# zerchen/AlignSDF

Hardware: AMD Instinct MI355X
Metric: meshes_per_sec_hand_plus_obj_N256 (higher is better)
Workload: dtype f32-class: 2 x f16 planes per operand (22 bit), 3 f16 MFMAs per product sum, f32 accumulate, every voxel <= 1e-5

## Files before the change

### alignsdf_amd/csrc/sdf_mlp_f16w_kernel.h

```cpp
#pragma once
#include "sdf_mlp_f16_kernel.h"

namespace asdf {

static_assert(ASDF16_STAGE_KB == 16 && ASDF16_MIX_SPLIT && ASDF16_EPI_STEPS && ASDF16_DMA_PER_KB && ASDF16_PRELOAD && ASDF16_LOADS_FIRST &&
                  ASDF16_PIN_ACC,
              "the W form is written for the shipped schedule of the split-half kernel");

#define ASDF_MFMA16W(a, b, c) __builtin_amdgcn_mfma_f32_16x16x32_f16((a), (b), (c), 0, 0, 0)
#define ASDF_MFMA4W(a, b, c) __builtin_amdgcn_mfma_f32_16x16x4f32((a), (b), (c), 0, 0, 0)

__device__ __forceinline__ f32x4 acc_get4(const f32x16& a, int o) {
  f32x4 v;
  v[0] = a[o]; v[1] = a[o + 1]; v[2] = a[o + 2]; v[3] = a[o + 3];
  return v;
}
__device__ __forceinline__ void acc_set4(f32x16& a, int o, const f32x4& v) { a[o] = v[0]; a[o + 1] = v[1]; a[o + 2] = v[2]; a[o + 3] = v[3]; }

__device__ __forceinline__ f32x16 load_bias16w(const float* tile_words, int lane) {
  const int q = lane >> 4;
  const float* w0 = tile_words + (q & 1) * 16 + 4 * (q >> 1);
  int dup = 0;
  asm volatile("" : "+v"(dup));
  const float* w1 = w0 + dup;
  f32x16 r;
  acc_set4(r, 0, *reinterpret_cast<const f32x4*>(w0)); acc_set4(r, 4, *reinterpret_cast<const f32x4*>(w0 + 8));
  acc_set4(r, 8, *reinterpret_cast<const f32x4*>(w1)); acc_set4(r, 12, *reinterpret_cast<const f32x4*>(w1 + 8));
  return r;
}

__device__ __forceinline__ void pin_acc_w(f32x16& acc) {
#pragma unroll
  for (int o = 0; o < 16; o += 4) {
    f32x4 q;
    q[0] = acc[o]; q[1] = acc[o + 1]; q[2] = acc[o + 2]; q[3] = acc[o + 3];
    asm volatile("" : "+a"(q));
    acc[o] = q[0]; acc[o + 1] = q[1]; acc[o + 2] = q[2]; acc[o + 3] = q[3];
  }
}

#ifndef ASDF16_W_M0_CLOBBER
#define ASDF16_W_M0_CLOBBER 1
#endif
template <int P>
__device__ __forceinline__ void dma_piece_w(const float* src, unsigned dst) {
#if ASDF16_W_M0_CLOBBER
  asm volatile(
      "s_mov_b32 m0, %1\n\t"
      "s_nop 0\n\t"
      "global_load_lds_dwordx4 %0, off offset:%c2"
      :
      : "v"(src + (P >> 2) * 1024), "s"(dst + (P >> 2) * 4096), "i"((P & 3) * 1024)
      : "memory", "m0");
#else
  dma_piece<P>(src, dst);
#endif
}

template <int KB, int Q, int SLOT, int ABL, class Pre, class Epi>
__device__ __forceinline__ void stage16w(f32x16& acc, const h8 (&xh)[KB], const h8 (&xl)[KB], const float* ring, const float* next_src,
                                         unsigned lds_ring_base, int lane, int wave, h8 (&ah)[S16<2>::kPrefetch], h8 (&al)[S16<2>::kPrefetch],
                                         Pre&& pre, Epi&& epi) {
  using SG = S16<2>;
  constexpr int PF = SG::kPrefetch;
  constexpr int BKB = ASDF16_BARRIER_KB;
  constexpr int nslot = (SLOT + kRing - 1) % kRing;
  static_assert(KB == 32 || KB == 16, "records per tile");
  static_assert(kS16Kb - BKB >= SG::kPieces, "one LDS-DMA piece per record behind the barrier");
  const float* src = next_src + wave * SG::kWaveFloats + lane * 4;
  const unsigned dst = lds_ring_base + (nslot * SG::kFloats + wave * SG::kWaveFloats) * 4;
  const h8* cur = reinterpret_cast<const h8*>(ring + SLOT * SG::kFloats) + lane;
  const h8* nxt = reinterpret_cast<const h8*>(ring + ((SLOT + 1) % kRing) * SG::kFloats) + lane;
  h8 bufh[kS16Kb + PF], bufl[kS16Kb + PF];
#pragma unroll
  for (int i = 0; i < PF; ++i) { bufh[i] = ah[i]; bufl[i] = al[i]; }
#pragma unroll
  for (int kb = 0; kb < kS16Kb; ++kb) {
    if (kb == BKB && !(ABL & 1)) {
      asm volatile("s_waitcnt vmcnt(8)" ::: "memory");
      if (!(ABL & 16)) __builtin_amdgcn_s_barrier();
    }
    bufh[kb + PF] = kb + PF < kS16Kb ? cur[((kb + PF) * 2 + 0) * 64] : nxt[((kb + PF - kS16Kb) * 2 + 0) * 64];
    bufl[kb + PF] = kb + PF < kS16Kb ? cur[((kb + PF) * 2 + 1) * 64] : nxt[((kb + PF - kS16Kb) * 2 + 1) * 64];
    pre(kb);
    __builtin_amdgcn_sched_barrier(0);
    const int ri = Q * kS16Kb + kb;
    const int xb = KB == 32 ? 2 * (ri % 16) : (ri & ~1), o = (KB == 32 ? ri / 16 : (ri & 1)) * 4;
    const bool snake = ri & 1;
    const int xa = xb + (snake ? 1 : 0), xc = xb + (snake ? 0 : 1);
#pragma unroll
    for (int j = 0; j < 3; ++j) {
      f32x4 s0 = acc_get4(acc, o), s1 = acc_get4(acc, 8 + o);
      f32x4& sa = snake ? s1 : s0;
      f32x4& sb = snake ? s0 : s1;
      if (j == 0) { sa = ASDF_MFMA16W(bufh[kb], xl[xa], sa); sa = ASDF_MFMA16W(bufl[kb], xh[xa], sa); }
      if (j == 1) { sa = ASDF_MFMA16W(bufh[kb], xh[xa], sa); sb = ASDF_MFMA16W(bufh[kb], xl[xc], sb); }
      if (j == 2) { sb = ASDF_MFMA16W(bufl[kb], xh[xc], sb); sb = ASDF_MFMA16W(bufh[kb], xh[xc], sb); }
      acc_set4(acc, o, s0); acc_set4(acc, 8 + o, s1);
      const int m = j == 2 ? kb - BKB : -1;
      if (!(ABL & 1) && !(ABL & 32) && m >= 0 && m < SG::kPieces) {
        if (m == 0) dma_piece_w<0>(src, dst);
        else if (m == 1) dma_piece_w<1>(src, dst);
        else if (m == 2) dma_piece_w<2>(src, dst);
        else if (m == 3) dma_piece_w<3>(src, dst);
        else if (m == 4) dma_piece_w<4>(src, dst);
        else if (m == 5) dma_piece_w<5>(src, dst);
        else if (m == 6) dma_piece_w<6>(src, dst);
        else dma_piece_w<7>(src, dst);
        __builtin_amdgcn_sched_barrier(0);
      }
      epi(kb, j);
      __builtin_amdgcn_sched_barrier(0);
    }
    __builtin_amdgcn_sched_barrier(0);
  }
#pragma unroll
  for (int i = 0; i < PF; ++i) { ah[i] = bufh[kS16Kb + i]; al[i] = bufl[kS16Kb + i]; }
}

template <int ABL = 0, bool SUB = false>
__device__ __forceinline__ void sdf_mlp_f16w_body(const DecodeParams& p) {
  using CL = CstLayout<2>;
  using SG = S16<2>;
  static_assert(lds_bytes_f16(2, 2) <= 160 * 1024, "LDS budget");
  extern __shared__ __attribute__((aligned(16))) float smem[];
  float* ring = smem;
  float* cst = smem + SG::kRingFloats;

  const int tid = threadIdx.x;
  const int lane = tid & 63;
  const int wave = __builtin_amdgcn_readfirstlane(tid >> 6);
  const int half = lane >> 5;

  float lat_vs = p.vs, lat_o0 = p.o0, lat_o1 = p.o1, lat_o2 = p.o2;
  if (p.lattice) { lat_o0 = p.lattice[0]; lat_o1 = p.lattice[1]; lat_o2 = p.lattice[2]; lat_vs = p.lattice[3]; }
  long long npts = p.P;
  if (SUB) { const long long c = *p.count_dev; npts = c < npts ? c : npts; }
  const long long ntiles = (npts + kWgPts - 1) / kWgPts;
  if ((long long)blockIdx.x >= ntiles) return;

  const unsigned lds_ring_base = (unsigned)(size_t)(__attribute__((address_space(3))) float*)ring;
  if (!SUB && p.status && p.mode != kPointList && blockIdx.x == 0 && tid == 0) reinterpret_cast<long long*>(p.status + ASDF_STATUS_CLOCK)[0] = clock64();

#pragma unroll 1
  for (int slot = 0; slot < p.num_mlps; ++slot) {
    const int head = p.first_mlp + slot;
    const float* hc = cst;
    int* wrec = reinterpret_cast<int*>(cst + CL::kFloats) + wave * kWrecInts;
    if (lane < kWrecInts) wrec[lane] = lane >= 16 ? 0 : ((lane & 7) < 3 ? 0x7fffffff : ((lane & 7) < 6 ? -1 : 0));
    asm volatile("s_waitcnt vmcnt(0)" ::: "memory");
    __syncthreads();
    {
      const f32x4* src4 = reinterpret_cast<const f32x4*>(p.cst + (size_t)head * CL::kFloats);
      for (int i = tid; i < CL::kFloats / 4; i += 256) reinterpret_cast<f32x4*>(cst)[i] = src4[i];
    }
    const float* sbase0 = p.stream + (size_t)kStagesAll * kStageFloats + (size_t)head * kS16Head * SG::kFloats;
#pragma unroll
    for (int s = 0; s < ((ABL & 33) ? kRing : kRing - 1); ++s) {
      const float* src = sbase0 + (size_t)s * SG::kFloats + wave * SG::kWaveFloats + lane * 4;
      const unsigned dst = lds_ring_base + (s * SG::kFloats + wave * SG::kWaveFloats) * 4;
#pragma unroll
      for (int c = 0; c < SG::kPieces; ++c) lds_dma16(src + c * 256, dst + c * 1024);
    }
    if (ABL & 33) asm volatile("s_waitcnt vmcnt(0)" ::: "memory");
    asm volatile("s_waitcnt vmcnt(16)" ::: "memory");
    __syncthreads();
    h8 ah[SG::kPrefetch], al[SG::kPrefetch];
#pragma unroll
    for (int i = 0; i < SG::kPrefetch; ++i) {
      ah[i] = (reinterpret_cast<const h8*>(ring) + lane)[(i * 2 + 0) * 64];
      al[i] = (reinterpret_cast<const h8*>(ring) + lane)[(i * 2 + 1) * 64];
    }
    const float mul1 = hc[CL::kB4 + 2], mul2 = hc[CL::kB4 + 3], mul0 = hc[CL::kB4 + 4];
    int audit_from = 0x7fffffff;
    if (SUB && p.audit) audit_from = p.audit_from ? *p.audit_from : 0;
    auto bias_at = [&](int off, int t) -> f32x16 { return load_bias16w(hc + off + t * 32, lane); };
    auto pt_word = [&](int off, int t, int fh) -> float {
      return hc[off + (t * 2 + (lane >> 5)) * 64 + ((lane >> 4) & 1) * 32 + 16 * fh + (lane & 15)];
    };

#pragma unroll 1
    for (long long tile = blockIdx.x; tile < ntiles; tile += gridDim.x) {
      const long long pi = tile * kWgPts + wave * kWavePts + (lane & 31);
      const bool valid = pi < npts;
      const long long po = SUB ? (valid ? (long long)p.idx[pi] : 0) : pi;
      float x0 = 0.f, x1 = 0.f, x2 = 0.f;
      if (SUB) {
        grid_point(po, p.N, p.grid_mode, lat_vs, lat_o0, lat_o1, lat_o2, x0, x1, x2);
      } else if (p.mode == kPointList) {
        if (valid) { x0 = p.xyz[pi * 3 + 0]; x1 = p.xyz[pi * 3 + 1]; x2 = p.xyz[pi * 3 + 2]; }
      } else {
        grid_point(valid ? pi : 0, p.N, p.mode, lat_vs, lat_o0, lat_o1, lat_o2, x0, x1, x2);
      }
      float amax = 0.0f, amax1 = 0.0f, amax2 = 0.0f;
      float bq[2];
      {
        const int q = lane >> 4;
#pragma unroll
        for (int g = 0; g < 2; ++g) {
          const int src = (lane & 15) + 16 * g;
          const float c0 = __shfl(x0, src), c1 = __shfl(x1, src), c2 = __shfl(x2, src);
          bq[g] = q == 0 ? c0 : q == 1 ? c1 : q == 2 ? c2 : 0.0f;
        }
      }
      auto pt_mfma = [&](f32x16& a, const float* af) {
#pragma unroll
        for (int fh = 0; fh < 2; ++fh)
#pragma unroll
          for (int g = 0; g < 2; ++g) acc_set4(a, 8 * g + 4 * fh, ASDF_MFMA4W(af[fh], bq[g], acc_get4(a, 8 * g + 4 * fh)));
      };
      const float* sbase = sbase0;
      asm volatile("" : "+s"(sbase));
      auto src_of = [&](int s) -> const float* {
        return sbase + (size_t)(s < kS16Head ? s : s - kS16Head) * SG::kFloats;
      };

      f32x16 acc1[2], acc2[2], acc3[2];
      float pf2[2];
      float w4c[2], w4n[2];
      constexpr int kPreKb = ASDF16_PRE_KB;
      static_assert(kPreKb >= kEpiShift + kEpiChunks, "preload K-block inside the epilogue slots");
      auto load_pf2 = [&](int t) { pf2[0] = pt_word(CL::kA2, t, 0); pf2[1] = pt_word(CL::kA2, t, 1); };
      auto load_w4 = [&](int t, int c) {
        const int wq = lane >> 4;
        const float* w4 = hc + CL::kW4 + (t * 2 + (wq & 1)) * 16 + 4 * (2 * ((c >> 1) & 1) + (wq >> 1)) + 2 * (c & 1);
        w4n[0] = w4[0]; w4n[1] = w4[1];
      };
      auto next_w4 = [&]() { w4c[0] = w4n[0]; w4c[1] = w4n[1]; };

      h8 h0h[2 * kTilesHidden], h0l[2 * kTilesHidden];
      f32x16 acc0[2];
      float pf0[2][2];
      auto l0_load = [&](int t) {
        acc0[t & 1] = bias_at(CL::kC0, t);
        pf0[t & 1][0] = pt_word(CL::kA0, t, 0); pf0[t & 1][1] = pt_word(CL::kA0, t, 1);
      };
      constexpr int kL0Front = kS16Kb / 2;
      l0_load(0);
      acc1[0] = bias_at(CL::kB1, 0);
#pragma unroll
      for (int t = 0; t < kL0Front; ++t) {
        l0_load(t + 1);
        __builtin_amdgcn_sched_barrier(0);
        f32x16 acc = acc0[t & 1];
        pt_mfma(acc, pf0[t & 1]);
        split_tile<2, 1, true>(acc, acc, mul0, h0h[2 * t], h0l[2 * t], h0h[2 * t + 1], h0l[2 * t + 1], amax);
        __builtin_amdgcn_sched_barrier(0);
      }

#define ASDF_STAGE16W(KB, Q, SLOT, ACC, XH, XL, SIDX, PRE, EPI) \
  stage16w<KB, Q, SLOT, ABL>(ACC, XH, XL, ring, src_of((SIDX) + 3), lds_ring_base, lane, wave, ah, al, PRE, EPI)

      float er[2] = {0.0f, 0.0f};
      h8 h1h[2 * kTilesL1], h1l[2 * kTilesL1];
      if (ABL & 4) for (int t = 0; t < 2 * kTilesL1; ++t) { h1h[t] = h0h[t]; h1l[t] = h0l[t]; }
#pragma unroll
      for (int t = 0; t < kTilesL1; ++t) {
        f32x16& acc = acc1[t & 1];
        auto pre = [&](int kb) {
          const int c = kb - kEpiShift;
          if (t == 0 && c >= 0 && c + 1 < kEpiChunks) l0_load(kL0Front + c + 1);
        };
        auto epi = [&](int kb, int g) {
          const int c = kb - kEpiShift;
          if (c < 0 || c >= kEpiChunks) return;
          if (t == 0) {
            const int T = kL0Front + c;
            if (g == 0) pt_mfma(acc0[T & 1], pf0[T & 1]);
#pragma unroll
            for (int e = 0; e < 8; ++e)
              if (e / 3 == g) split_part<2, 1, true>(acc0[T & 1], acc0[T & 1], mul0, h0h[2 * T], h0l[2 * T], h0h[2 * T + 1], h0l[2 * T + 1], amax, e);
            return;
          }
          if (ABL & 4) { asm volatile("" :: "v"(acc1[(t - 1) & 1])); return; }
          if (g == 0) pin_acc_w(acc1[(t - 1) & 1]);
          split_part<2, 1, true>(acc1[(t - 1) & 1], acc1[(t - 1) & 1], mul1, h1h[2 * (t - 1)], h1l[2 * (t - 1)], h1h[2 * (t - 1) + 1],
                                 h1l[2 * (t - 1) + 1], amax1, c, -1, g, er);
        };
        auto pre_last = [&](int c) {
          if (c != kPreKb) return;
          if (t + 1 < kTilesL1) acc1[(t + 1) & 1] = bias_at(CL::kB1, t + 1);
          else { acc2[0] = bias_at(CL::kC2, 0); load_pf2(0); }
        };
        if (t & 1) {
          ASDF_STAGE16W(32, 0, 2, acc, h0h, h0l, t * 2 + 0, pre, epi);
          ASDF_STAGE16W(32, 1, 3, acc, h0h, h0l, t * 2 + 1, pre_last, NoOp16());
        } else {
          ASDF_STAGE16W(32, 0, 0, acc, h0h, h0l, t * 2 + 0, pre, epi);
          ASDF_STAGE16W(32, 1, 1, acc, h0h, h0l, t * 2 + 1, pre_last, NoOp16());
        }
      }

      h8 h2h[2 * kTilesHidden], h2l[2 * kTilesHidden];
      if (ABL & 4) for (int t = 0; t < 2 * kTilesHidden; ++t) { h2h[t] = h0h[t]; h2l[t] = h0l[t]; }
      auto l2_tile = [&](int t, auto slot_tag) {
        constexpr int SLOT = decltype(slot_tag)::value;
        f32x16& acc = acc2[t & 1];
        pt_mfma(acc, pf2);
        auto epi = [&](int kb, int g) {
          const int c = kb - kEpiShift;
          if (c < 0 || c >= kEpiChunks) return;
          if (ABL & 4) { asm volatile("" :: "v"(acc2[(t + 1) & 1]), "v"(acc1[1])); return; }
          if (t > 0) {
            if (g == 0) pin_acc_w(acc2[(t - 1) & 1]);
            split_part<2, 1, true>(acc2[(t - 1) & 1], acc2[(t - 1) & 1], mul2, h2h[2 * (t - 1)], h2l[2 * (t - 1)], h2h[2 * (t - 1) + 1],
                                   h2l[2 * (t - 1) + 1], amax2, c, -1, g, er);
          } else {
            if (g == 0) pin_acc_w(acc1[(kTilesL1 - 1) & 1]);
            split_part<2, 1, true>(acc1[(kTilesL1 - 1) & 1], acc1[(kTilesL1 - 1) & 1], mul1, h1h[2 * kTilesL1 - 2], h1l[2 * kTilesL1 - 2],
                                   h1h[2 * kTilesL1 - 1], h1l[2 * kTilesL1 - 1], amax1, c, -1, g, er);
          }
        };
        auto pre_last = [&](int c) {
          if (c != kPreKb) return;
          if (t + 1 < kTilesHidden) { acc2[(t + 1) & 1] = bias_at(CL::kC2, t + 1); load_pf2(t + 1); }
          else acc3[0] = bias_at(CL::kB3, 0);
        };
        constexpr int S0 = 256 / kS16Kb;
        ASDF_STAGE16W(16, 0, SLOT, acc, h1h, h1l, S0 + t, pre_last, epi);
      };
#pragma unroll
      for (int tt = 0; tt < kTilesHidden / 4; ++tt) {
        l2_tile(4 * tt + 0, std::integral_constant<int, 0>());
        l2_tile(4 * tt + 1, std::integral_constant<int, 1>());
        l2_tile(4 * tt + 2, std::integral_constant<int, 2>());
        l2_tile(4 * tt + 3, std::integral_constant<int, 3>());
      }

      float part = 0.0f, partg = 0.0f;
      auto dot_w4_part = [&](const f32x16& a, int c, int only = -1) {
#pragma unroll
        for (int r = 0; r < 2; ++r) {
          if (only >= 0 && only != r) continue;
          const float v = __int_as_float(max(__float_as_int(a[2 * c + r]), 0));
          if (c < 4) part = fmaf(v, w4c[r], part);
          else partg = fmaf(v, w4c[r], partg);
        }
      };
#pragma unroll
      for (int t = 0; t < kTilesHidden; ++t) {
        f32x16& acc = acc3[t & 1];
        auto pre = [&](int kb) {
          const int c = kb - kEpiShift;
          if (t > 0 && c >= 0 && c + 1 < kEpiChunks) load_w4(t - 1, c + 1);
        };
        auto epi = [&](int kb, int g) {
          const int c = kb - kEpiShift;
          if (c < 0 || c >= kEpiChunks) return;
          if (ABL & 4) { asm volatile("" :: "v"(acc3[(t + 1) & 1]), "v"(acc2[1])); return; }
          if (t > 0) {
            if (g == 0) pin_acc_w(acc3[(t - 1) & 1]);
            if (g < 2) dot_w4_part(acc3[(t - 1) & 1], c, g);
            else next_w4();
          } else {
            if (g == 0) pin_acc_w(acc2[(kTilesHidden - 1) & 1]);
            split_part<2, 1, true>(acc2[(kTilesHidden - 1) & 1], acc2[(kTilesHidden - 1) & 1], mul2, h2h[2 * kTilesHidden - 2],
                                   h2l[2 * kTilesHidden - 2], h2h[2 * kTilesHidden - 1], h2l[2 * kTilesHidden - 1], amax2, c, -1, g, er);
          }
        };
        auto pre_last = [&](int c) {
          if (c != kPreKb) return;
          if (t + 1 < kTilesHidden) acc3[(t + 1) & 1] = bias_at(CL::kB3, t + 1);
          load_w4(t, 0);
          next_w4();
        };
        constexpr int S0 = 512 / kS16Kb;
        if (t & 1) {
          ASDF_STAGE16W(32, 0, 2, acc, h2h, h2l, S0 + t * 2 + 0, pre, epi);
          ASDF_STAGE16W(32, 1, 3, acc, h2h, h2l, S0 + t * 2 + 1, pre_last, NoOp16());
        } else {
          ASDF_STAGE16W(32, 0, 0, acc, h2h, h2l, S0 + t * 2 + 0, pre, epi);
          ASDF_STAGE16W(32, 1, 1, acc, h2h, h2l, S0 + t * 2 + 1, pre_last, NoOp16());
        }
      }
#pragma unroll
      for (int c = 0; c < kEpiChunks; ++c) {
        if (c + 1 < kEpiChunks) load_w4(kTilesHidden - 1, c + 1);
        dot_w4_part(acc3[(kTilesHidden - 1) & 1], c);
        next_w4();
      }
#undef ASDF_STAGE16W
      part += __shfl_xor(part, 16); partg += __shfl_xor(partg, 16);
      part += __shfl_xor(part, 32); partg += __shfl_xor(partg, 32);
      part = (lane & 16) ? partg : part;
      const float pre = part + hc[CL::kB4];
      const float sdf = tanhf(pre);
      const bool is_hand = head == 0;
      if (SUB) {
        int dm = 0, da = 0, flips = 0, na = 0;
        float sq = 0.0f;
        if (valid && half == 0) {
          const bool aud = p.audit && pi >= (long long)audit_from;
          float* out = is_hand ? p.sdf0 : p.sdf1;
          if (out) {
            const float before = out[po];
            const int d = __float_as_int(fabsf(sdf - before));
            if (aud) { da = max(da, d); flips += ((before < 0.0f) != (sdf < 0.0f)) ? 1 : 0; ++na; sq += (sdf - before) * (sdf - before); }
            else dm = max(dm, d);
            if (!aud || p.audit_from) out[po] = sdf;
          }
        }
#pragma unroll
        for (int m = 32; m >= 1; m >>= 1) {
          dm = max(dm, __shfl_xor(dm, m)); da = max(da, __shfl_xor(da, m));
          flips += __shfl_xor(flips, m); na += __shfl_xor(na, m);
          if (p.audit) sq += __shfl_xor(sq, m);
        }
        if (lane == 0) {
          if (p.status && dm) atomicMax(p.status + ASDF_STATUS_MAX_ERR, dm);
          if (p.audit && na) {
            atomicMax(p.audit + kAuditMaxErr, da); if (flips) atomicAdd(p.audit + kAuditFlips, flips); atomicAdd(p.audit + kAuditEvals, na);
            atomicAdd(reinterpret_cast<float*>(p.audit + kAuditSumSq), sq);
          }
        }
      } else if (valid && half == 0) {
        float* out = is_hand ? p.sdf0 : p.sdf1;
        if (out) out[po] = sdf;
      }
      amax *= mul0; amax1 *= mul1; amax2 *= mul2;
      const bool act_over = !(fmaxf(amax, fmaxf(amax1, amax2)) < 65504.0f);
      const int bad = (valid && (act_over || !(fabsf(sdf) <= 1.0f))) ? 1 : 0;
      if (p.status) {
        const int m0 = wave_max_i32(valid ? __float_as_int(amax) : 0), m1 = wave_max_i32(valid ? __float_as_int(amax1) : 0),
                  m2 = wave_max_i32(valid ? __float_as_int(amax2) : 0);
        if (lane == 0) { wrec[16] = max(wrec[16], m0); wrec[17] = max(wrec[17], m1); wrec[18] = max(wrec[18], m2); }
      }
      if (!SUB && p.bbox && p.mode != kPointList) {
        const bool neg = valid && half == 0 && sdf < p.neg_thr;
        int extra = bad;
        if (__any(neg || extra != 0)) {
          int i0, i1, i2;
          lattice_ijk(pi, p.N, i0, i1, i2);
          int a0 = neg ? i0 : 0x7fffffff, a1 = neg ? i1 : 0x7fffffff, a2 = neg ? i2 : 0x7fffffff;
          int b0 = neg ? i0 : -1, b1 = neg ? i1 : -1, b2 = neg ? i2 : -1, n = neg ? 1 : 0;
#pragma unroll
          for (int m = 32; m >= 1; m >>= 1) {
            a0 = min(a0, __shfl_xor(a0, m)); a1 = min(a1, __shfl_xor(a1, m)); a2 = min(a2, __shfl_xor(a2, m));
            b0 = max(b0, __shfl_xor(b0, m)); b1 = max(b1, __shfl_xor(b1, m)); b2 = max(b2, __shfl_xor(b2, m));
            n += __shfl_xor(n, m);
            extra += __shfl_xor(extra, m);
          }
          if (lane == 0 && (n | extra)) {
            wrec[0] = min(wrec[0], a0); wrec[1] = min(wrec[1], a1); wrec[2] = min(wrec[2], a2);
            wrec[3] = max(wrec[3], b0); wrec[4] = max(wrec[4], b1); wrec[5] = max(wrec[5], b2);
            wrec[6] += n; wrec[7] += extra;
          }
        }
      } else {
        const unsigned long long m = __ballot(bad);
        if (m && lane == 0) wrec[7] += __popcll(m);
      }
    }

    if (lane == 0) {
      if (p.bbox && p.mode != kPointList) {
        int* out = p.bbox + (head == 0 ? 0 : ASDF_BOX_STRIDE);
        if (wrec[6]) {
          atomicMin(out + ASDF_BOX_MIN + 0, wrec[0]); atomicMin(out + ASDF_BOX_MIN + 1, wrec[1]); atomicMin(out + ASDF_BOX_MIN + 2, wrec[2]);
          atomicMax(out + ASDF_BOX_MAX + 0, wrec[3]); atomicMax(out + ASDF_BOX_MAX + 1, wrec[4]); atomicMax(out + ASDF_BOX_MAX + 2, wrec[5]);
          atomicAdd(out + ASDF_BOX_COUNT, wrec[6]);
        }
        if (wrec[7]) atomicAdd(p.bbox + (head == 0 ? ASDF_BOX_RANGE : ASDF_BOX_STRIDE + ASDF_BOX_RANGE), wrec[7]);
      }
      if (p.status) {
        if (wrec[7]) atomicAdd(p.status + ASDF_STATUS_RANGE, wrec[7]);
        int* peak = p.status + ASDF_STATUS_PEAK + ASDF_STATUS_PEAK_STRIDE * head;
        atomicMax(peak + 0, wrec[16]); atomicMax(peak + 1, wrec[17]); atomicMax(peak + 2, wrec[18]);
      }
    }
  }
  asm volatile("s_waitcnt vmcnt(0)" ::: "memory");
  if (!SUB && p.status && p.mode != kPointList && blockIdx.x == 0 && tid == 0) reinterpret_cast<long long*>(p.status + ASDF_STATUS_CLOCK)[1] = clock64();
}


}
```

Measured before the change: 14.11.

## Defer per-tile output epilogue into next tile's layer-1 stage slots

Moves the final layer-4 dot product, tanh, store, peak tracking and bbox fold for each tile out of the tile's own tail. It now runs inside the epilogue hooks of the next tile's first layer-1 stage, with a drain after the loop for the last tile. The aim is to hide the serial scalar tail behind MFMA work of the following tile instead of leaving the matrix units idle. In exchange, acc3 and the peak values must stay live across iterations, which raises register pressure. The change also adds segment timing markers under a macro.

```diff
diff --git a/alignsdf_amd/csrc/sdf_mlp_f16w_kernel.h b/alignsdf_amd/csrc/sdf_mlp_f16w_kernel.h
--- a/alignsdf_amd/csrc/sdf_mlp_f16w_kernel.h
+++ b/alignsdf_amd/csrc/sdf_mlp_f16w_kernel.h
@@ -17,9 +17,9 @@
 }
 __device__ __forceinline__ void acc_set4(f32x16& a, int o, const f32x4& v) { a[o] = v[0]; a[o + 1] = v[1]; a[o + 2] = v[2]; a[o + 3] = v[3]; }
 
-__device__ __forceinline__ f32x16 load_bias16w(const float* tile_words, int lane) {
-  const int q = lane >> 4;
-  const float* w0 = tile_words + (q & 1) * 16 + 4 * (q >> 1);
+__device__ __forceinline__ int bias_lane_words(int lane) { const int q = lane >> 4; return (q & 1) * 16 + 4 * (q >> 1); }
+__device__ __forceinline__ f32x16 load_bias16w(const float* tile_words, int lane_words) {
+  const float* w0 = tile_words + lane_words;
   int dup = 0;
   asm volatile("" : "+v"(dup));
   const float* w1 = w0 + dup;
@@ -56,6 +56,10 @@
   dma_piece<P>(src, dst);
 #endif
 }
+
+#ifndef ASDF16_W_XTILE
+#define ASDF16_W_XTILE 1
+#endif
 
 template <int KB, int Q, int SLOT, int ABL, class Pre, class Epi>
 __device__ __forceinline__ void stage16w(f32x16& acc, const h8 (&xh)[KB], const h8 (&xl)[KB], const float* ring, const float* next_src,
@@ -174,13 +178,137 @@
     const float mul1 = hc[CL::kB4 + 2], mul2 = hc[CL::kB4 + 3], mul0 = hc[CL::kB4 + 4];
     int audit_from = 0x7fffffff;
     if (SUB && p.audit) audit_from = p.audit_from ? *p.audit_from : 0;
-    auto bias_at = [&](int off, int t) -> f32x16 { return load_bias16w(hc + off + t * 32, lane); };
+    int bias_lane = bias_lane_words(lane);
+    auto bias_at = [&](int off, int t) -> f32x16 { return load_bias16w(hc + off + t * 32, bias_lane); };
     auto pt_word = [&](int off, int t, int fh) -> float {
       return hc[off + (t * 2 + (lane >> 5)) * 64 + ((lane >> 4) & 1) * 32 + 16 * fh + (lane & 15)];
     };
 
+    constexpr bool XT = ASDF16_W_XTILE && !SUB;
+    f32x16 acc3[2];
+    float part = 0.0f, partg = 0.0f;
+    float pamax = 0.0f, pamax1 = 0.0f, pamax2 = 0.0f;
+    if (XT) {
+#pragma unroll
+      for (int r = 0; r < 16; ++r) acc3[1][r] = 0.0f;
+    }
+    float w4c[2], w4n[2];
+    auto load_w4 = [&](int t, int c) {
+      const int wq = lane >> 4;
+      const float* w4 = hc + CL::kW4 + (t * 2 + (wq & 1)) * 16 + 4 * (2 * ((c >> 1) & 1) + (wq >> 1)) + 2 * (c & 1);
+      w4n[0] = w4[0]; w4n[1] = w4[1];
+    };
+    auto next_w4 = [&]() { w4c[0] = w4n[0]; w4c[1] = w4n[1]; };
+    auto dot_w4_part = [&](const f32x16& a, int c, int only = -1) {
+#pragma unroll
+      for (int r = 0; r < 2; ++r) {
+        if (only >= 0 && only != r) continue;
+        const float v = __int_as_float(max(__float_as_int(a[2 * c + r]), 0));
+        if (c < 4) part = fmaf(v, w4c[r], part);
+        else partg = fmaf(v, w4c[r], partg);
+      }
+    };
+    const bool is_hand = head == 0;
+    float sdf = 0.0f;
+    int bad = 0;
+    auto tail_value = [&]() {
+      part += __shfl_xor(part, 16); partg += __shfl_xor(partg, 16);
+      part += __shfl_xor(part, 32); partg += __shfl_xor(partg, 32);
+      part = (lane & 16) ? partg : part;
+      const float pre = part + hc[CL::kB4];
+      sdf = tanhf(pre);
+    };
+    auto tail_store = [&](long long pi, bool valid, long long po) {
+      if (SUB) {
+        int dm = 0, da = 0, flips = 0, na = 0;
+        float sq = 0.0f;
+        if (valid && half == 0) {
+          const bool aud = p.audit && pi >= (long long)audit_from;
+          float* out = is_hand ? p.sdf0 : p.sdf1;
+          if (out) {
+            const float before = out[po];
+            const int d = __float_as_int(fabsf(sdf - before));
+            if (aud) { da = max(da, d); flips += ((before < 0.0f) != (sdf < 0.0f)) ? 1 : 0; ++na; sq += (sdf - before) * (sdf - before); }
+            else dm = max(dm, d);
+            if (!aud || p.audit_from) out[po] = sdf;
+          }
+        }
+#pragma unroll
+        for (int m = 32; m >= 1; m >>= 1) {
+          dm = max(dm, __shfl_xor(dm, m)); da = max(da, __shfl_xor(da, m));
+          flips += __shfl_xor(flips, m); na += __shfl_xor(na, m);
+          if (p.audit) sq += __shfl_xor(sq, m);
+        }
+        if (lane == 0) {
+          if (p.status && dm) atomicMax(p.status + ASDF_STATUS_MAX_ERR, dm);
+          if (p.audit && na) {
+            atomicMax(p.audit + kAuditMaxErr, da); if (flips) atomicAdd(p.audit + kAuditFlips, flips); atomicAdd(p.audit + kAuditEvals, na);
+            atomicAdd(reinterpret_cast<float*>(p.audit + kAuditSumSq), sq);
+          }
+        }
+      } else if (valid && half == 0) {
+        float* out = is_hand ? p.sdf0 : p.sdf1;
+        if (out) out[po] = sdf;
+      }
+    };
+    auto tail_peaks = [&](bool valid, float amax, float amax1, float amax2) {
+      amax *= mul0; amax1 *= mul1; amax2 *= mul2;
+      const bool act_over = !(fmaxf(amax, fmaxf(amax1, amax2)) < 65504.0f);
+      bad = (valid && (act_over || !(fabsf(sdf) <= 1.0f))) ? 1 : 0;
+      if (p.status) {
+        const int m0 = wave_max_i32(valid ? __float_as_int(amax) : 0), m1 = wave_max_i32(valid ? __float_as_int(amax1) : 0),
+                  m2 = wave_max_i32(valid ? __float_as_int(amax2) : 0);
+        if (lane == 0) { wrec[16] = max(wrec[16], m0); wrec[17] = max(wrec[17], m1); wrec[18] = max(wrec[18], m2); }
+      }
+    };
+    auto tail_fold = [&](long long pi, bool valid) {
+      if (!SUB && p.bbox && p.mode != kPointList) {
+        const bool neg = valid && half == 0 && sdf < p.neg_thr;
+        int extra = bad;
+        if (__any(neg || extra != 0)) {
+          int i0, i1, i2;
+          lattice_ijk(pi, p.N, i0, i1, i2);
+          int a0 = neg ? i0 : 0x7fffffff, a1 = neg ? i1 : 0x7fffffff, a2 = neg ? i2 : 0x7fffffff;
+          int b0 = neg ? i0 : -1, b1 = neg ? i1 : -1, b2 = neg ? i2 : -1, n = neg ? 1 : 0;
+#pragma unroll
+          for (int m = 32; m >= 1; m >>= 1) {
+            a0 = min(a0, __shfl_xor(a0, m)); a1 = min(a1, __shfl_xor(a1, m)); a2 = min(a2, __shfl_xor(a2, m));
+            b0 = max(b0, __shfl_xor(b0, m)); b1 = max(b1, __shfl_xor(b1, m)); b2 = max(b2, __shfl_xor(b2, m));
+            n += __shfl_xor(n, m);
+            extra += __shfl_xor(extra, m);
+          }
+          if (lane == 0 && (n | extra)) {
+            wrec[0] = min(wrec[0], a0); wrec[1] = min(wrec[1], a1); wrec[2] = min(wrec[2], a2);
+            wrec[3] = max(wrec[3], b0); wrec[4] = max(wrec[4], b1); wrec[5] = max(wrec[5], b2);
+            wrec[6] += n; wrec[7] += extra;
+          }
+        }
+      } else {
+        const unsigned long long m = __ballot(bad);
+        if (m && lane == 0) wrec[7] += __popcll(m);
+      }
+    };
+    auto tail_bare = [&](long long pi, bool valid, long long po, float amax, float amax1, float amax2) {
+#pragma unroll
+      for (int c = 0; c < kEpiChunks; ++c) {
+        if (c + 1 < kEpiChunks) load_w4(kTilesHidden - 1, c + 1);
+        dot_w4_part(acc3[(kTilesHidden - 1) & 1], c);
+        next_w4();
+      }
+      tail_value();
+      tail_store(pi, valid, po);
+      tail_peaks(valid, amax, amax1, amax2);
+      tail_fold(pi, valid);
+    };
+
+    long long tile = blockIdx.x;
 #pragma unroll 1
-    for (long long tile = blockIdx.x; tile < ntiles; tile += gridDim.x) {
+    for (; tile < ntiles; tile += gridDim.x) {
+#ifdef ASDF16_SEGMENT_TIMES
+      long long seg_t[8];
+#endif
+      ASDF16_MARK(0);
+      asm volatile("" : "+v"(bias_lane));
       const long long pi = tile * kWgPts + wave * kWavePts + (lane & 31);
       const bool valid = pi < npts;
       const long long po = SUB ? (valid ? (long long)p.idx[pi] : 0) : pi;
@@ -203,6 +331,7 @@
           bq[g] = q == 0 ? c0 : q == 1 ? c1 : q == 2 ? c2 : 0.0f;
         }
       }
+      ASDF16_MARK(7);
       auto pt_mfma = [&](f32x16& a, const float* af) {
 #pragma unroll
         for (int fh = 0; fh < 2; ++fh)
@@ -215,18 +344,11 @@
         return sbase + (size_t)(s < kS16Head ? s : s - kS16Head) * SG::kFloats;
       };
 
-      f32x16 acc1[2], acc2[2], acc3[2];
+      f32x16 acc1[2], acc2[2];
       float pf2[2];
-      float w4c[2], w4n[2];
       constexpr int kPreKb = ASDF16_PRE_KB;
       static_assert(kPreKb >= kEpiShift + kEpiChunks, "preload K-block inside the epilogue slots");
       auto load_pf2 = [&](int t) { pf2[0] = pt_word(CL::kA2, t, 0); pf2[1] = pt_word(CL::kA2, t, 1); };
-      auto load_w4 = [&](int t, int c) {
-        const int wq = lane >> 4;
-        const float* w4 = hc + CL::kW4 + (t * 2 + (wq & 1)) * 16 + 4 * (2 * ((c >> 1) & 1) + (wq >> 1)) + 2 * (c & 1);
-        w4n[0] = w4[0]; w4n[1] = w4[1];
-      };
-      auto next_w4 = [&]() { w4c[0] = w4n[0]; w4c[1] = w4n[1]; };
 
       h8 h0h[2 * kTilesHidden], h0l[2 * kTilesHidden];
       f32x16 acc0[2];
@@ -247,6 +369,7 @@
         split_tile<2, 1, true>(acc, acc, mul0, h0h[2 * t], h0l[2 * t], h0h[2 * t + 1], h0l[2 * t + 1], amax);
         __builtin_amdgcn_sched_barrier(0);
       }
+      ASDF16_MARK(1);
 
 #define ASDF_STAGE16W(KB, Q, SLOT, ACC, XH, XL, SIDX, PRE, EPI) \
   stage16w<KB, Q, SLOT, ABL>(ACC, XH, XL, ring, src_of((SIDX) + 3), lds_ring_base, lane, wave, ah, al, PRE, EPI)
@@ -287,9 +410,39 @@
           ASDF_STAGE16W(32, 1, 3, acc, h0h, h0l, t * 2 + 1, pre_last, NoOp16());
         } else {
           ASDF_STAGE16W(32, 0, 0, acc, h0h, h0l, t * 2 + 0, pre, epi);
-          ASDF_STAGE16W(32, 1, 1, acc, h0h, h0l, t * 2 + 1, pre_last, NoOp16());
-        }
-      }
+          if constexpr (XT) {
+            if (t == 0) {
+              const long long ppi = (tile - gridDim.x) * kWgPts + wave * kWavePts + (lane & 31);
+              const bool pvalid = ppi >= 0 && ppi < npts;
+              auto pre_tail = [&](int kb) {
+                pre_last(kb);
+                const int c = kb - kEpiShift;
+                if (c >= -1 && c + 1 < kEpiChunks) load_w4(kTilesHidden - 1, c + 1);
+              };
+              auto epi_tail = [&](int kb, int g) {
+                const int c = kb - kEpiShift;
+                if (c < 0) { if (g == 2) next_w4(); return; }
+                if (c < kEpiChunks) {
+                  if (g == 0) pin_acc_w(acc3[(kTilesHidden - 1) & 1]);
+                  if (g < 2) dot_w4_part(acc3[(kTilesHidden - 1) & 1], c, g);
+                  else next_w4();
+                  return;
+                }
+                if (c == kEpiChunks && g == 0) tail_value();
+                if (c == kEpiChunks && g == 1) tail_store(ppi, pvalid, ppi);
+                if (c == kEpiChunks + 2 && g == 0) tail_peaks(pvalid, pamax, pamax1, pamax2);
+                if (c == kEpiChunks + 3 && g == 0) tail_fold(ppi, pvalid);
+              };
+              ASDF_STAGE16W(32, 1, 1, acc, h0h, h0l, t * 2 + 1, pre_tail, epi_tail);
+            } else {
+              ASDF_STAGE16W(32, 1, 1, acc, h0h, h0l, t * 2 + 1, pre_last, NoOp16());
+            }
+          } else {
+            ASDF_STAGE16W(32, 1, 1, acc, h0h, h0l, t * 2 + 1, pre_last, NoOp16());
+          }
+        }
+      }
+      ASDF16_MARK(2);
 
       h8 h2h[2 * kTilesHidden], h2l[2 * kTilesHidden];
       if (ABL & 4) for (int t = 0; t < 2 * kTilesHidden; ++t) { h2h[t] = h0h[t]; h2l[t] = h0l[t]; }
@@ -326,17 +479,9 @@
         l2_tile(4 * tt + 2, std::integral_constant<int, 2>());
         l2_tile(4 * tt + 3, std::integral_constant<int, 3>());
       }
-
-      float part = 0.0f, partg = 0.0f;
-      auto dot_w4_part = [&](const f32x16& a, int c, int only = -1) {
-#pragma unroll
-        for (int r = 0; r < 2; ++r) {
-          if (only >= 0 && only != r) continue;
-          const float v = __int_as_float(max(__float_as_int(a[2 * c + r]), 0));
-          if (c < 4) part = fmaf(v, w4c[r], part);
-          else partg = fmaf(v, w4c[r], partg);
-        }
-      };
+      ASDF16_MARK(3);
+
+      part = 0.0f; partg = 0.0f;
 #pragma unroll
       for (int t = 0; t < kTilesHidden; ++t) {
         f32x16& acc = acc3[t & 1];
@@ -361,6 +506,7 @@
         auto pre_last = [&](int c) {
           if (c != kPreKb) return;
           if (t + 1 < kTilesHidden) acc3[(t + 1) & 1] = bias_at(CL::kB3, t + 1);
+          if (XT && t + 1 == kTilesHidden) return;
           load_w4(t, 0);
           next_w4();
         };
@@ -373,83 +519,22 @@
           ASDF_STAGE16W(32, 1, 1, acc, h2h, h2l, S0 + t * 2 + 1, pre_last, NoOp16());
         }
       }
-#pragma unroll
-      for (int c = 0; c < kEpiChunks; ++c) {
-        if (c + 1 < kEpiChunks) load_w4(kTilesHidden - 1, c + 1);
-        dot_w4_part(acc3[(kTilesHidden - 1) & 1], c);
-        next_w4();
-      }
 #undef ASDF_STAGE16W
-      part += __shfl_xor(part, 16); partg += __shfl_xor(partg, 16);
-      part += __shfl_xor(part, 32); partg += __shfl_xor(partg, 32);
-      part = (lane & 16) ? partg : part;
-      const float pre = part + hc[CL::kB4];
-      const float sdf = tanhf(pre);
-      const bool is_hand = head == 0;
-      if (SUB) {
-        int dm = 0, da = 0, flips = 0, na = 0;
-        float sq = 0.0f;
-        if (valid && half == 0) {
-          const bool aud = p.audit && pi >= (long long)audit_from;
-          float* out = is_hand ? p.sdf0 : p.sdf1;
-          if (out) {
-            const float before = out[po];
-            const int d = __float_as_int(fabsf(sdf - before));
-            if (aud) { da = max(da, d); flips += ((before < 0.0f) != (sdf < 0.0f)) ? 1 : 0; ++na; sq += (sdf - before) * (sdf - before); }
-            else dm = max(dm, d);
-            if (!aud || p.audit_from) out[po] = sdf;
-          }
-        }
-#pragma unroll
-        for (int m = 32; m >= 1; m >>= 1) {
-          dm = max(dm, __shfl_xor(dm, m)); da = max(da, __shfl_xor(da, m));
-          flips += __shfl_xor(flips, m); na += __shfl_xor(na, m);
-          if (p.audit) sq += __shfl_xor(sq, m);
-        }
-        if (lane == 0) {
-          if (p.status && dm) atomicMax(p.status + ASDF_STATUS_MAX_ERR, dm);
-          if (p.audit && na) {
-            atomicMax(p.audit + kAuditMaxErr, da); if (flips) atomicAdd(p.audit + kAuditFlips, flips); atomicAdd(p.audit + kAuditEvals, na);
-            atomicAdd(reinterpret_cast<float*>(p.audit + kAuditSumSq), sq);
-          }
-        }
-      } else if (valid && half == 0) {
-        float* out = is_hand ? p.sdf0 : p.sdf1;
-        if (out) out[po] = sdf;
-      }
-      amax *= mul0; amax1 *= mul1; amax2 *= mul2;
-      const bool act_over = !(fmaxf(amax, fmaxf(amax1, amax2)) < 65504.0f);
-      const int bad = (valid && (act_over || !(fabsf(sdf) <= 1.0f))) ? 1 : 0;
-      if (p.status) {
-        const int m0 = wave_max_i32(valid ? __float_as_int(amax) : 0), m1 = wave_max_i32(valid ? __float_as_int(amax1) : 0),
-                  m2 = wave_max_i32(valid ? __float_as_int(amax2) : 0);
-        if (lane == 0) { wrec[16] = max(wrec[16], m0); wrec[17] = max(wrec[17], m1); wrec[18] = max(wrec[18], m2); }
-      }
-      if (!SUB && p.bbox && p.mode != kPointList) {
-        const bool neg = valid && half == 0 && sdf < p.neg_thr;
-        int extra = bad;
-        if (__any(neg || extra != 0)) {
-          int i0, i1, i2;
-          lattice_ijk(pi, p.N, i0, i1, i2);
-          int a0 = neg ? i0 : 0x7fffffff, a1 = neg ? i1 : 0x7fffffff, a2 = neg ? i2 : 0x7fffffff;
-          int b0 = neg ? i0 : -1, b1 = neg ? i1 : -1, b2 = neg ? i2 : -1, n = neg ? 1 : 0;
-#pragma unroll
-          for (int m = 32; m >= 1; m >>= 1) {
-            a0 = min(a0, __shfl_xor(a0, m)); a1 = min(a1, __shfl_xor(a1, m)); a2 = min(a2, __shfl_xor(a2, m));
-            b0 = max(b0, __shfl_xor(b0, m)); b1 = max(b1, __shfl_xor(b1, m)); b2 = max(b2, __shfl_xor(b2, m));
-            n += __shfl_xor(n, m);
-            extra += __shfl_xor(extra, m);
-          }
-          if (lane == 0 && (n | extra)) {
-            wrec[0] = min(wrec[0], a0); wrec[1] = min(wrec[1], a1); wrec[2] = min(wrec[2], a2);
-            wrec[3] = max(wrec[3], b0); wrec[4] = max(wrec[4], b1); wrec[5] = max(wrec[5], b2);
-            wrec[6] += n; wrec[7] += extra;
-          }
-        }
-      } else {
-        const unsigned long long m = __ballot(bad);
-        if (m && lane == 0) wrec[7] += __popcll(m);
-      }
+      ASDF16_MARK(4);
+      if (XT) { pamax = amax; pamax1 = amax1; pamax2 = amax2; }
+      else tail_bare(pi, valid, po, amax, amax1, amax2);
+      ASDF16_MARK(5);
+#ifdef ASDF16_SEGMENT_TIMES
+      if (blockIdx.x == 0 && wave == 0 && lane == 0 && slot == 0 && tile == (long long)blockIdx.x + 2 * gridDim.x)
+        { for (int k = 0; k < 6; ++k) g_seg[k] = (unsigned long long)seg_t[k]; g_seg[7] = (unsigned long long)seg_t[7]; }
+      if (blockIdx.x == 0 && wave == 0 && lane == 0 && slot == 0 && tile == (long long)blockIdx.x + 3 * gridDim.x) g_seg[6] = (unsigned long long)seg_t[0];
+#endif
+    }
+    if (XT) {
+      const long long ppi = (tile - gridDim.x) * kWgPts + wave * kWavePts + (lane & 31);
+      load_w4(kTilesHidden - 1, 0);
+      next_w4();
+      tail_bare(ppi, ppi < npts, ppi, pamax, pamax1, pamax2);
     }
 
     if (lane == 0) {
```

New measurement: 14.01. About the same (-0.7%).
